# CFGpp-diffusion/CFGpp

Measured on NVIDIA B200. Metric: images/sec (device-timed) SDXL 1024x1024 NFE=50 ddim_cfg++, higher is better.
Workload: dtype f16

## Files before the change

cfgpp_b200/csrc/attention.cu:

```cuda
#include <cmath>
#include <cstdlib>
#include <cstring>

#include "attention.cuh"
#include "common.cuh"

namespace cfgpp {

void attn_configure();
void xattn_configure();
bool xattn_applicable(const AttnOp& op);
void run_xattn_op(const AttnOp& op, cudaStream_t stream);
void attn_persist_configure();
bool attn_persist_applicable(const AttnOp& op);
void run_attn_persist_op(const AttnOp& op, cudaStream_t stream);

namespace {

constexpr int BQ = 128;
constexpr int BKV = 128;
constexpr int ATOM_BYTES = 128 * 64 * 2;
constexpr int kThreads = 384;
constexpr uint32_t TMEM_COLS = 512;
constexpr float kRescaleThreshold = 8.0f;
constexpr int kDefaultPoly = 0;
constexpr int kDefaultRowsumMma = 0;
constexpr int kDefaultPbuf = 1;

template <int HD, int NQT, int KS, bool RS = false, int PB = 1>
struct ACfg {
  static constexpr int NA = HD / 64;
  static constexpr int TILE_BYTES = NA * ATOM_BYTES;
  static constexpr int P_BYTES = 2 * ATOM_BYTES;
  static constexpr int OW = HD + (RS ? 16 : 0);
  static constexpr int SMEM_BYTES =
      TILE_BYTES * (NQT + 2 * KS) + P_BYTES * NQT * PB + (RS ? ATOM_BYTES : 0) + 1024 + 256;
  static constexpr uint32_t O_COL = NQT * 128;
  static_assert(!RS || HD == 64, "the ones column is implemented for head dim 64");
  static_assert(NQT * 128 + NQT * OW <= 512, "TMEM overflow");
  static_assert(SMEM_BYTES <= 232448, "shared memory overflow");
};

template <int HD, int NQT, int KS, int POLY, bool RS, int PB>
__global__ void __launch_bounds__(kThreads, 1)
attn_kernel(const AttnParams p, const __grid_constant__ CUtensorMap map_q, const __grid_constant__ CUtensorMap map_k,
            const __grid_constant__ CUtensorMap map_v) {
  using A = ACfg<HD, NQT, KS, RS, PB>;
  constexpr int OW = A::OW;
  constexpr int TILE_BYTES = A::TILE_BYTES;
  constexpr int NA = A::NA;
  constexpr uint32_t O_COL = A::O_COL;
  extern __shared__ uint8_t smem_raw[];
  const uint32_t raw_addr = smem_u32(smem_raw);
  uint8_t* smem = smem_raw + (((raw_addr + 1023u) & ~1023u) - raw_addr);
  uint8_t* sQ = smem;
  uint8_t* sK = sQ + NQT * TILE_BYTES;
  uint8_t* sV = sK + KS * TILE_BYTES;
  uint8_t* sP = sV + KS * TILE_BYTES;
  uint8_t* sOnes = sP + NQT * PB * A::P_BYTES;
  uint64_t* bars = reinterpret_cast<uint64_t*>(sOnes + (RS ? ATOM_BYTES : 0));
  uint64_t* q_full = bars;
  uint64_t* k_full = q_full + 2;
  uint64_t* k_empty = k_full + KS;
  uint64_t* v_full = k_empty + KS;
  uint64_t* v_empty = v_full + KS;
  uint64_t* s_full = v_empty + KS;
  uint64_t* s_free = s_full + 2;
  uint64_t* p_full = s_free + 2;
  uint64_t* pv_done = p_full + 2 * PB;
  uint32_t* tmem_ptr_smem = reinterpret_cast<uint32_t*>(pv_done + 2 * PB);

  const int warp_idx = threadIdx.x >> 5;
  const int lane = threadIdx.x & 31;
  const int q0 = blockIdx.x * NQT * BQ;
  const int head = blockIdx.y;
  const int batch = blockIdx.z;
  const int n_tiles = (p.Nkv + BKV - 1) / BKV;
  const int n_qt = (NQT == 2 && q0 + BQ < p.Nq) ? 2 : 1;

  if (warp_idx == 0 && lane == 0) {
    tma_prefetch_desc(&map_q);
    tma_prefetch_desc(&map_k);
    tma_prefetch_desc(&map_v);
  }
  if (warp_idx == 1 && lane == 0) {
    for (int i = 0; i < 2; ++i) {
      mbar_init(&q_full[i], 1);
      mbar_init(&s_full[i], 1);
      mbar_init(&s_free[i], 128);
      for (int b = 0; b < PB; ++b) {
        mbar_init(&p_full[i * PB + b], 128);
        mbar_init(&pv_done[i * PB + b], 1);
      }
    }
    for (int i = 0; i < KS; ++i) {
      mbar_init(&k_full[i], 1);
      mbar_init(&k_empty[i], n_qt);
      mbar_init(&v_full[i], 1);
      mbar_init(&v_empty[i], n_qt);
    }
    fence_barrier_init();
  }
  if (warp_idx == 2) {
    tmem_alloc(tmem_ptr_smem, TMEM_COLS);
    tmem_relinquish();
  }
  if constexpr (RS) {
    if (warp_idx == 3) {
      for (int k = lane; k < 128; k += 32) {
        uint4* rowp = reinterpret_cast<uint4*>(sOnes + k * 128);
#pragma unroll
        for (int ch = 0; ch < 8; ++ch) rowp[ch] = make_uint4(ch == (k & 7) ? 0x00003C00u : 0u, 0u, 0u, 0u);
      }
      fence_proxy_async_smem();
    }
  }
  tc_fence_before();
  __syncthreads();
  tc_fence_after();
  const uint32_t tmem_base = *tmem_ptr_smem;
  pdl_launch_dependents();
  pdl_wait();

  if (warp_idx == 0) {
    if (lane == 0) {
      for (int qt = 0; qt < n_qt; ++qt) {
        mbar_arrive_expect_tx(&q_full[qt], TILE_BYTES);
        for (int a = 0; a < NA; ++a)
          tma_load_3d(sQ + qt * TILE_BYTES + a * ATOM_BYTES, &map_q, &q_full[qt], head * HD + a * 64, q0 + qt * BQ,
                      batch);
      }
      for (int j = 0; j < n_tiles; ++j) {
        const int s = j % KS;
        const uint32_t ph = (j / KS) & 1;
        mbar_wait(&k_empty[s], ph ^ 1);
        mbar_arrive_expect_tx(&k_full[s], TILE_BYTES);
        for (int a = 0; a < NA; ++a)
          tma_load_3d(sK + s * TILE_BYTES + a * ATOM_BYTES, &map_k, &k_full[s], head * HD + a * 64, j * BKV, batch);
        mbar_wait(&v_empty[s], ph ^ 1);
        mbar_arrive_expect_tx(&v_full[s], TILE_BYTES);
        for (int a = 0; a < NA; ++a)
          tma_load_3d(sV + s * TILE_BYTES + a * ATOM_BYTES, &map_v, &v_full[s], head * HD + a * 64, j * BKV, batch);
      }
    }
  } else if (warp_idx == 1) {
    if (lane == 0) {
      constexpr uint32_t idesc_qk = make_idesc_f16(128, BKV, 0, 0);
      constexpr uint32_t idesc_pv = make_idesc_f16(128, OW, 0, 1);
      auto issue_qk = [&](int qt, int j) {
#pragma unroll
        for (int a = 0; a < NA; ++a) {
          const uint64_t q_desc = make_sdesc_sw128(smem_u32(sQ + qt * TILE_BYTES + a * ATOM_BYTES), 1024, 0);
          const uint64_t k_desc = make_sdesc_sw128(smem_u32(sK + (j % KS) * TILE_BYTES + a * ATOM_BYTES), 1024, 0);
#pragma unroll
          for (int k = 0; k < 4; ++k)
            umma_f16(tmem_base + qt * BKV, q_desc + 2 * k, k_desc + 2 * k, idesc_qk, (a | k) != 0 ? 1u : 0u);
        }
        umma_commit(&s_full[qt]);
      };
      auto issue_pv = [&](int qt, int j) {
        const uint32_t v_addr = smem_u32(sV + (j % KS) * TILE_BYTES);
        const uint64_t v_desc = make_sdesc_sw128(v_addr, 1024, RS ? (smem_u32(sOnes) - v_addr) : ATOM_BYTES);
        const uint8_t* pbuf = sP + (qt * PB + (j % PB)) * A::P_BYTES;
#pragma unroll
        for (int k = 0; k < BKV / 16; ++k) {
          const uint64_t p_desc = make_sdesc_sw128(smem_u32(pbuf + (k >> 2) * ATOM_BYTES), 1024, 0) + 2 * (k & 3);
          umma_f16(tmem_base + O_COL + qt * OW, p_desc, v_desc + 128 * k, idesc_pv, (j | k) != 0 ? 1u : 0u);
        }
        umma_commit(&pv_done[qt * PB + (j % PB)]);
      };
      for (int qt = 0; qt < n_qt; ++qt) mbar_wait(&q_full[qt], 0);
      mbar_wait(&k_full[0], 0);
      tc_fence_after();
      for (int qt = 0; qt < n_qt; ++qt) {
        issue_qk(qt, 0);
// ... 16 lines not shown
            progressed = true;
          }
          j = next_qk[qt];
          if (j < n_tiles && mbar_try_wait(&s_free[qt], (j - 1) & 1) && mbar_try_wait(&k_full[j % KS], (j / KS) & 1)) {
            tc_fence_after();
            issue_qk(qt, j);
            umma_commit(&k_empty[j % KS]);
            ++next_qk[qt];
            --remaining;
            progressed = true;
          }
        }
        if (progressed) {
          t_start = clock64();
        } else if (clock64() - t_start > 4000000000LL) {
          printf("cfgpp: attention MMA issuer stalled (block %d,%d,%d)\n", blockIdx.x, blockIdx.y, blockIdx.z);
          __trap();
        }
      }
    }
  } else if (warp_idx >= 4) {
    const int qt = (warp_idx - 4) >> 2;
    if (qt < n_qt) {
      const int qw = warp_idx & 3;
      const int row = qw * 32 + lane;
      const uint32_t lane_off = static_cast<uint32_t>(qw * 32) << 16;
      const uint32_t s_addr = tmem_base + qt * BKV + lane_off;
      const uint32_t o_addr = tmem_base + O_COL + qt * OW + lane_off;
      uint8_t* prow0 = sP + qt * PB * A::P_BYTES + row * 128;
      const float c = p.scale_log2e;
      float m_ref = -INFINITY, l_run = 0.f;

      for (int j = 0; j < n_tiles; ++j) {
        const int valid = p.Nkv - j * BKV;
        mbar_wait(&s_full[qt], j & 1);
        tc_fence_after();
        uint32_t s[128];
#pragma unroll
        for (int g = 0; g < 4; ++g) tmem_ld_x32(s_addr + g * 32, *reinterpret_cast<uint32_t(*)[32]>(&s[g * 32]));
        tmem_ld_wait();
        tc_fence_before();
        mbar_arrive(&s_free[qt]);
        if (valid < BKV) {
#pragma unroll
          for (int i = 0; i < 128; ++i)
            if (i >= valid) s[i] = 0xff800000u;
        }
        float mxc[8];
#pragma unroll
        for (int k8 = 0; k8 < 8; ++k8) mxc[k8] = fmaxf(__uint_as_float(s[k8]), __uint_as_float(s[8 + k8]));
#pragma unroll
        for (int i = 16; i < 128; i += 16) {
#pragma unroll
          for (int k8 = 0; k8 < 8; ++k8) mxc[k8] = fmax3(mxc[k8], __uint_as_float(s[i + k8]), __uint_as_float(s[i + 8 + k8]));
        }
        const float mx = fmax3(fmax3(mxc[0], mxc[1], mxc[2]), fmax3(mxc[3], mxc[4], mxc[5]), fmaxf(mxc[6], mxc[7]));
        float alpha = 1.0f;
        bool need = false;
        if (j == 0) {
          m_ref = mx;
        } else if ((mx - m_ref) * c > kRescaleThreshold) {
          alpha = fast_exp2((m_ref - mx) * c);
          m_ref = mx;
          need = true;
        }
        uint8_t* prow = prow0 + (j % PB) * A::P_BYTES;
        if (j >= PB) {
          mbar_wait(&pv_done[qt * PB + (j % PB)], ((j - PB) / PB) & 1);
          tc_fence_after();
        }
        if (j > 0 && __any_sync(0xffffffffu, need)) {
          if constexpr (PB > 1) {
            mbar_wait(&pv_done[qt * PB + ((j - 1) % PB)], ((j - 1) / PB) & 1);
            tc_fence_after();
          }
#pragma unroll 1
          for (int h = 0; h < OW / 16; ++h) {
            uint32_t o[16];
            tmem_ld_x16(o_addr + h * 16, o);
            tmem_ld_wait();
#pragma unroll
            for (int d = 0; d < 16; ++d) o[d] = __float_as_uint(__uint_as_float(o[d]) * alpha);
            tmem_st_x16(o_addr + h * 16, o);
          }
          tmem_st_wait();
          l_run *= alpha;
        }
        const float mc = m_ref * c;
        float rs0 = 0.f, rs1 = 0.f;
#pragma unroll
        for (int g = 0; g < 16; ++g) {
          uint32_t pk[4];
#pragma unroll
          for (int e = 0; e < 4; ++e) {
            const float x0 = __uint_as_float(s[g * 8 + 2 * e]) * c - mc;
            const float x1 = __uint_as_float(s[g * 8 + 2 * e + 1]) * c - mc;
            constexpr int kP = POLY > 0 ? POLY : 1;
            const bool poly0 = POLY > 0 && ((g * 8 + 2 * e) % kP) == kP - 1;
            const bool poly1 = POLY > 0 && ((g * 8 + 2 * e + 1) % kP) == kP - 1;
            const float p0 = poly0 ? exp2_poly(x0) : fast_exp2(x0);
            const float p1 = poly1 ? exp2_poly(x1) : fast_exp2(x1);
            if constexpr (!RS) {
              rs0 += p0;
              rs1 += p1;
            }
            pk[e] = pack_half2(p0, p1);
          }
          const int half_idx = g >> 3;
          const int ch = (g & 7) ^ (row & 7);
          *reinterpret_cast<uint4*>(prow + half_idx * ATOM_BYTES + ch * 16) = make_uint4(pk[0], pk[1], pk[2], pk[3]);
        }
        l_run += rs0 + rs1;
        tc_fence_before();
        fence_proxy_async_smem();
        mbar_arrive(&p_full[qt * PB + (j % PB)]);
      }
      mbar_wait(&pv_done[qt * PB + ((n_tiles - 1) % PB)], ((n_tiles - 1) / PB) & 1);
      tc_fence_after();
      if constexpr (RS) {
        uint32_t lcol[16];
        tmem_ld_x16(o_addr + HD, lcol);
        tmem_ld_wait();
        l_run = __uint_as_float(lcol[0]);
      }
      const float inv_l = 1.0f / l_run;
      const int qrow = q0 + qt * BQ + row;
      __half* dst = p.out + (static_cast<size_t>(batch) * p.Nq + qrow) * p.ldo + head * HD;
#pragma unroll 1
      for (int h = 0; h < HD / 32; ++h) {
        uint32_t o[32];
        tmem_ld_x32(o_addr + h * 32, o);
        tmem_ld_wait();
        if (qrow < p.Nq) {
#pragma unroll
          for (int i = 0; i < 4; ++i) {
            uint4 w;
            w.x = pack_half2(__uint_as_float(o[8 * i + 0]) * inv_l, __uint_as_float(o[8 * i + 1]) * inv_l);
            w.y = pack_half2(__uint_as_float(o[8 * i + 2]) * inv_l, __uint_as_float(o[8 * i + 3]) * inv_l);
            w.z = pack_half2(__uint_as_float(o[8 * i + 4]) * inv_l, __uint_as_float(o[8 * i + 5]) * inv_l);
            w.w = pack_half2(__uint_as_float(o[8 * i + 6]) * inv_l, __uint_as_float(o[8 * i + 7]) * inv_l);
            reinterpret_cast<uint4*>(dst + h * 32)[i] = w;
          }
        }
      }
    }
  }

  tc_fence_before();
  __syncthreads();
  if (warp_idx == 2) {
    tc_fence_after();
    tmem_dealloc(tmem_base, TMEM_COLS);
  }
}

CUtensorMap make_head_map(const __half* base, int ld, int B, int N, int cols) {
  uint64_t dims[3] = {(uint64_t)cols, (uint64_t)N, (uint64_t)B};
  uint64_t strides[2] = {(uint64_t)ld * 2, (uint64_t)N * ld * 2};
  uint32_t box[3] = {64, 128, 1};
  return make_tmap_f16(base, 3, dims, strides, box);
}

template <int HD, int NQT, int KS, int POLY = 0, bool RS = false, int PB = 1>
void configure_one() {
  CFGPP_CHECK_CUDA(cudaFuncSetAttribute(attn_kernel<HD, NQT, KS, POLY, RS, PB>,
                                        cudaFuncAttributeMaxDynamicSharedMemorySize,
                                        ACfg<HD, NQT, KS, RS, PB>::SMEM_BYTES));
}

template <int HD, int NQT, int KS, int POLY = 0, bool RS = false, int PB = 1>
void launch(const AttnOp& op, cudaStream_t stream) {
  dim3 grid((op.p.Nq + NQT * BQ - 1) / (NQT * BQ), op.p.H, op.p.B);
  launch_pdl(attn_kernel<HD, NQT, KS, POLY, RS, PB>, grid, dim3(kThreads), ACfg<HD, NQT, KS, RS, PB>::SMEM_BYTES, stream,
             op.p, op.map_q, op.map_k, op.map_v);
}

int attn_pbuf() {
  static int v = -1;
  if (v < 0) {
    const char* e = std::getenv("CFGPP_ATTN_PBUF");
    v = e ? atoi(e) : kDefaultPbuf;
    if (v != 1 && v != 2) v = kDefaultPbuf;
  }
  return v;
}

bool attn_rowsum_mma() {
  static int v = -1;
  if (v < 0) {
    const char* e = std::getenv("CFGPP_ATTN_ROWSUM_MMA");
    v = e ? (e[0] == '1' ? 1 : 0) : kDefaultRowsumMma;
  }
  return v == 1;
}

int attn_poly() {
  static int v = -1;
  if (v < 0) {
    const char* e = std::getenv("CFGPP_ATTN_POLY");
    v = e ? atoi(e) : kDefaultPoly;
    if (v != 0 && v != 8 && v != 4 && v != 3) v = kDefaultPoly;
  }
  return v;
}

}

int attn_padded_head_dim(int head_dim) { return ((head_dim + 63) / 64) * 64; }

AttnOp make_attn_op(const __half* q, int ldq, const __half* k, int ldk, const __half* v, int ldv, __half* out,
                    int ldo, int B, int H, int Nq, int Nkv, int head_dim) {
  AttnOp op{};
  CFGPP_REQUIRE(Nkv >= 1 && Nq >= 1, "empty attention");
  CFGPP_REQUIRE(ldo % 8 == 0, "ldo must be a multiple of 8");
  CFGPP_REQUIRE(head_dim >= 8 && head_dim <= 192, "attention supports head_dim <= 192");
  const int hdp = attn_padded_head_dim(head_dim);
  op.hd_pad = hdp;
  op.head_dim = head_dim;
  op.p.B = B; op.p.H = H; op.p.Nq = Nq; op.p.Nkv = Nkv; op.p.ldo = ldo; op.p.out = out;
  op.p.scale_log2e = (1.0f / sqrtf(static_cast<float>(head_dim))) * 1.4426950408889634f;
  op.map_q = make_head_map(q, ldq, B, Nq, H * hdp);
  op.map_k = make_head_map(k, ldk, B, Nkv, H * hdp);
  op.map_v = make_head_map(v, ldv, B, Nkv, H * hdp);
  return op;
}

void attn_configure() {
  static bool done = false;
  if (done) return;
  configure_one<64, 2, 3>();
  configure_one<64, 2, 3, 8>();
  configure_one<64, 2, 3, 4>();
  configure_one<64, 2, 3, 3>();
  configure_one<64, 2, 3, 0, true>();
  configure_one<64, 2, 2, 0, false, 2>();
  configure_one<128, 1, 2>();
  configure_one<192, 1, 1>();
  xattn_configure();
  attn_persist_configure();
  done = true;
}

void run_attn_op(const AttnOp& op, cudaStream_t stream) {
  attn_configure();
  static const bool no_x = [] {
    const char* e = std::getenv("CFGPP_NO_XATTN");
    return e != nullptr && e[0] == '1';
  }();
  if (!no_x && xattn_applicable(op)) return run_xattn_op(op, stream);
  static const bool use_p = [] {
    const char* e = std::getenv("CFGPP_PATTN");
    return e != nullptr && e[0] == '1';
  }();
  if (use_p && attn_persist_applicable(op)) return run_attn_persist_op(op, stream);
  attn_configure();
  switch (op.hd_pad) {
    case 64:
      if (attn_pbuf() == 2) return launch<64, 2, 2, 0, false, 2>(op, stream);
      if (attn_rowsum_mma()) return launch<64, 2, 3, 0, true>(op, stream);
      switch (attn_poly()) {
        case 8: return launch<64, 2, 3, 8>(op, stream);
        case 4: return launch<64, 2, 3, 4>(op, stream);
        case 3: return launch<64, 2, 3, 3>(op, stream);
        default: return launch<64, 2, 3>(op, stream);
      }
    case 128: return launch<128, 1, 2>(op, stream);
    case 192: return launch<192, 1, 1>(op, stream);
    default: throw Error(-1, "unsupported padded head dim");
  }
}

}
```

cfgpp_b200/csrc/attention.cuh:

```cuda
#pragma once
#include "host.h"

namespace cfgpp {

struct AttnParams {
  int B, H, Nq, Nkv;
  int ldo;
  __half* out;
  float scale_log2e;
};

struct AttnOp {
  CUtensorMap map_q, map_k, map_v;
  AttnParams p;
  int hd_pad;
  int head_dim;
  double flops() const { return 4.0 * p.B * p.H * (double)p.Nq * p.Nkv * head_dim; }
};

int attn_padded_head_dim(int head_dim);
AttnOp make_attn_op(const __half* q, int ldq, const __half* k, int ldk, const __half* v, int ldv, __half* out,
                    int ldo, int B, int H, int Nq, int Nkv, int head_dim = 64);
void run_attn_op(const AttnOp& op, cudaStream_t stream);

}
```

cfgpp_b200/csrc/capi_ops.cu:

```cuda
#include "capi_util.h"
#include "attention.cuh"
#include "gemm.cuh"
#include "ops.cuh"
#include "../../include/cfgpp_b200.h"

using namespace cfgpp;

extern "C" {

CFGPP_API int cfgpp_op_linear(const void* a, int lda, const void* a2, int lda2, int k_split, const void* w, int M,
                              int N, int K, const void* bias, const void* addend, int ld_add,
                              int add_rows_per_group, void* out, int ldc, int geglu, int force_bn, void* stream) {
  return guarded([&] {
    GemmOp op = make_linear_op((const __half*)a, lda, (const __half*)a2, lda2, k_split, (const __half*)w, M, N, K,
                               (const __half*)bias, (const __half*)addend, ld_add, add_rows_per_group, (__half*)out,
                               ldc, geglu != 0, force_bn);
    run_gemm_op(op, (cudaStream_t)stream);
  });
}

CFGPP_API int cfgpp_dbg_linear_timeline(const void* a, int lda, const void* w, int M, int N, int K, const void* bias,
                                        const void* addend, void* out, int force_bn, int iters,
                                        unsigned long long* host_out , int* grid_out, void* stream) {
  return guarded([&] {
// ... 3 lines not shown
    CFGPP_CHECK_CUDA(cudaMalloc(&d, sizeof(unsigned long long) * 16 * op.grid));
    CFGPP_CHECK_CUDA(cudaMemset(d, 0, sizeof(unsigned long long) * 16 * op.grid));
    op.p.timeline = d;
    for (int i = 0; i < iters; ++i) run_gemm_op(op, (cudaStream_t)stream);
    CFGPP_CHECK_CUDA(cudaStreamSynchronize((cudaStream_t)stream));
    CFGPP_CHECK_CUDA(cudaMemcpy(host_out, d, sizeof(unsigned long long) * 16 * op.grid, cudaMemcpyDeviceToHost));
    *grid_out = op.grid;
    cudaFree(d);
  });
}

CFGPP_API int cfgpp_op_conv3x3(const void* x, int B, int H, int W, int Cin, const void* w, int Cout, const void* bias,
                               const void* addend, int ld_add, int add_rows_per_group, void* out, int force_bn,
                               void* stream) {
  return guarded([&] {
    GemmOp op = make_conv3x3_op((const __half*)x, B, H, W, Cin, (const __half*)w, Cout, (const __half*)bias,
                                (const __half*)addend, ld_add, add_rows_per_group, (__half*)out, force_bn);
    run_gemm_op(op, (cudaStream_t)stream);
  });
}

CFGPP_API int cfgpp_op_conv3x3_s2(const void* x, int B, int H, int W, int Cin, const void* w, int Cout, const void* bias,
                                  int pad, void* out, void* stream) {
  return guarded([&] {
    GemmOp op = make_conv3x3_op((const __half*)x, B, H, W, Cin, (const __half*)w, Cout, (const __half*)bias, nullptr, 0, 1,
                                (__half*)out, 0, 2, pad);
    run_gemm_op(op, (cudaStream_t)stream);
  });
}

CFGPP_API int cfgpp_op_attention(const void* q, int ldq, const void* k, int ldk, const void* v, int ldv, void* out,
                                 int ldo, int B, int H, int Nq, int Nkv, int head_dim, void* stream) {
  return guarded([&] {
    AttnOp op = make_attn_op((const __half*)q, ldq, (const __half*)k, ldk, (const __half*)v, ldv, (__half*)out, ldo,
                             B, H, Nq, Nkv, head_dim);
    run_attn_op(op, (cudaStream_t)stream);
  });
}

CFGPP_API int cfgpp_op_groupnorm(const void* x1, int C1, const void* x2, int C2, int B, int HW, const void* gamma,
                                 const void* beta, float eps, int silu, void* out, void* stream) {
  return guarded([&] {
    float* partial = nullptr;
    CFGPP_CHECK_CUDA(cudaMalloc(&partial, gn_partial_floats(B, HW) * sizeof(float)));
    try {
      run_groupnorm((const __half*)x1, C1, (const __half*)x2, C2, B, HW, (const __half*)gamma, (const __half*)beta,
                    eps, silu != 0, partial, (__half*)out, (cudaStream_t)stream);
    } catch (...) {
      cudaFree(partial);
      throw;
    }
    CFGPP_CHECK_CUDA(cudaStreamSynchronize((cudaStream_t)stream));
    cudaFree(partial);
  });
}

CFGPP_API int cfgpp_op_layernorm(const void* x, int M, int C, const void* gamma, const void* beta, float eps,
                                 void* out, void* stream) {
  return guarded([&] {
    run_layernorm((const __half*)x, M, C, (const __half*)gamma, (const __half*)beta, eps, (__half*)out,
                  (cudaStream_t)stream);
  });
}

CFGPP_API int cfgpp_op_cfgpp_step(const void* eps_uc, const void* eps_c, int n, int method, int state_dtype,
                                  const cfgpp_step_coef* coef_host, void* z, void* aux, void* z0t_out,
                                  const void* noise_dev, void* stream) {
  return guarded([&] {
// ... 24 lines not shown
```

cfgpp_b200/csrc/common.cuh:

```cuda
#pragma once
#include <cuda.h>
#include <cuda_fp16.h>
#include <cuda_runtime.h>
#include <stdint.h>
#include <stdio.h>

namespace cfgpp {

#define CFGPP_DEVICE __device__ __forceinline__

CFGPP_DEVICE uint32_t smem_u32(const void* p) {
  return static_cast<uint32_t>(__cvta_generic_to_shared(p));
}

CFGPP_DEVICE void pdl_launch_dependents() { asm volatile("griddepcontrol.launch_dependents;" ::: "memory"); }
CFGPP_DEVICE void pdl_wait() { asm volatile("griddepcontrol.wait;" ::: "memory"); }

CFGPP_DEVICE void mbar_init(uint64_t* bar, uint32_t count) {
  asm volatile("mbarrier.init.shared::cta.b64 [%0], %1;" ::"r"(smem_u32(bar)), "r"(count));
}
CFGPP_DEVICE void fence_barrier_init() {
  asm volatile("fence.mbarrier_init.release.cluster;" ::: "memory");
}
CFGPP_DEVICE void mbar_arrive_expect_tx(uint64_t* bar, uint32_t bytes) {
// ... 272 lines not shown
  float e;
  asm("ex2.approx.ftz.f32 %0, %1;" : "=f"(e) : "f"(-az * az * 1.4426950408889634f));
  float p = 1.061405429f;
  p = fmaf(p, t, -1.453152027f);
  p = fmaf(p, t, 1.421413741f);
  p = fmaf(p, t, -0.284496736f);
  p = fmaf(p, t, 0.254829592f);
  const float q = p * t * e;
  return 0.5f * x * (x >= 0.f ? 2.0f - q : q);
}

CFGPP_DEVICE float fast_exp2(float x) {
  float y;
  asm("ex2.approx.ftz.f32 %0, %1;" : "=f"(y) : "f"(x));
  return y;
}

CFGPP_DEVICE float exp2_poly(float x) {
  x = fmaxf(x, -126.0f);
  const float t = x + 12582912.0f;
  const float r = x - (t - 12582912.0f);
  float p = 0.0551716648042202f;
  p = fmaf(p, r, 0.2426111251115799f);
  p = fmaf(p, r, 0.6932609677314758f);
  p = fmaf(p, r, 0.9999280571937561f);
  return __int_as_float(__float_as_int(p) + (__float_as_int(t) << 23));
}
CFGPP_DEVICE float fmax3(float a, float b, float c) {
  float d;
  asm("max.f32 %0, %1, %2, %3;" : "=f"(d) : "f"(a), "f"(b), "f"(c));
  return d;
}

CFGPP_DEVICE uint32_t pack_half2(float a, float b) {
  __half2 h = __floats2half2_rn(a, b);
  return *reinterpret_cast<uint32_t*>(&h);
}

}
```

cfgpp_b200/csrc/unet.cu:

```cuda
#include "unet.cuh"

#include <algorithm>
#include <cstdlib>
#include <cstring>

#include "common.cuh"

namespace cfgpp {

namespace {

__global__ void f32_to_f16_kernel(const float* __restrict__ in, __half* __restrict__ out, size_t n) {
  for (size_t i = blockIdx.x * static_cast<size_t>(blockDim.x) + threadIdx.x; i < n;
       i += static_cast<size_t>(gridDim.x) * blockDim.x)
    out[i] = __float2half_rn(in[i]);
}

__global__ void pack_conv3x3_kernel(const __half* __restrict__ in, __half* __restrict__ out, int Cout, int Cin) {
  const size_t n = static_cast<size_t>(Cout) * Cin * 9;
  for (size_t i = blockIdx.x * static_cast<size_t>(blockDim.x) + threadIdx.x; i < n;
       i += static_cast<size_t>(gridDim.x) * blockDim.x) {
    const int ci = i % Cin;
    const size_t t = i / Cin;
    const int tap = t % 9;
// ... 363 lines not shown
  add_gemm(prefix + ".conv1", make_conv3x3_op(normp, bnb_, H, W, Cin, packed_conv3x3(prefix + ".conv1.weight"), Cout,
                                              plain(prefix + ".conv1.bias"), temb_all_ + static_cast<size_t>(brow0_) * temb_total_ + temb_off, temb_total_, HW,
                                              h1p));
  add_step(prefix + ".norm2+silu", [=](cudaStream_t st) {
    run_groupnorm(h1p, Cout, nullptr, 0, NB, HW, g2, b2, eps, true, partial, normp, st);
  }, 2);
  const __half* residual = x1p;
  if (Cin != Cout) {
    add_gemm(prefix + ".conv_shortcut",
             make_linear_op(x1p, C1, x2p, C2, C1, plain(prefix + ".conv_shortcut.weight"), static_cast<int>(M), Cout,
                            Cin, plain(prefix + ".conv_shortcut.bias"), nullptr, 0, 1, s_sc->p, Cout, false));
    residual = s_sc->p;
  }
  add_gemm(prefix + ".conv2", make_conv3x3_op(normp, bnb_, H, W, Cout, packed_conv3x3(prefix + ".conv2.weight"), Cout,
                                              plain(prefix + ".conv2.bias"), residual, Cout, 1, out));
  return Act{out, Cout};
}

Unet::Act Unet::build_transformer(const std::string& prefix, Act x, int H, int W, int layers, int heads) {
  const int C = x.C;
  const int HW = H * W;
  const int Mi = bnb_ * HW;
  const size_t M = static_cast<size_t>(Mi);
  const int D = d_.cross_attention_dim;
  CFGPP_REQUIRE(C % heads == 0 && C / heads <= 192,
                "attention supports head_dim <= 192 (got " + std::to_string(C / std::max(heads, 1)) + ") at " + prefix);
  const int hd = C / heads;
  const int hdp = attn_padded_head_dim(hd);
  const int Cp = heads * hdp;
  Scratch* s_norm = scratch(btag_ + "norm", M * C);
  Scratch* s_tok = scratch(btag_ + "tokens", M * C);
  Scratch* s_qkv = scratch(btag_ + "qkv", M * 3 * Cp);
  Scratch* s_attn = scratch(btag_ + "attn", M * Cp);
  Scratch* s_q = scratch(btag_ + "q", M * Cp);
  Scratch* s_ff = scratch(btag_ + "ff", M * 4 * C);
  Scratch* s_stats[3];
  for (int i = 0; i < 3; ++i)
    s_stats[i] = scratch(btag_ + "lnstats" + std::to_string(i), static_cast<size_t>(32) * M * 2 * 2);
  __half* out = g_dry ? nullptr : alloc_act(M * C);
  const int Mkv = bnb_ * n_ctx_;
  if (g_dry) {
    raw(prefix + ".norm.weight"); raw(prefix + ".norm.bias"); raw(prefix + ".proj_in.weight");
    raw(prefix + ".proj_in.bias"); raw(prefix + ".proj_out.weight"); raw(prefix + ".proj_out.bias");
    for (int k = 0; k < layers; ++k) {
      const std::string b = prefix + ".transformer_blocks." + std::to_string(k);
      for (const char* n : {".norm1.weight", ".norm1.bias", ".norm2.weight", ".norm2.bias", ".norm3.weight",
                            ".norm3.bias", ".attn1.to_q.weight", ".attn1.to_k.weight", ".attn1.to_v.weight",
                            ".attn1.to_out.0.weight", ".attn1.to_out.0.bias", ".attn2.to_q.weight",
                            ".attn2.to_k.weight", ".attn2.to_v.weight", ".attn2.to_out.0.weight",
                            ".attn2.to_out.0.bias", ".ff.net.0.proj.weight", ".ff.net.0.proj.bias",
                            ".ff.net.2.weight", ".ff.net.2.bias"})
        raw(b + n);
      workspace_bytes_ += static_cast<size_t>(Mkv) * 2 * Cp * sizeof(__half);
    }
    workspace_bytes_ += M * C * sizeof(__half);
    return Act{nullptr, C};
  }
  const int NB = bnb_;
  float* partial = bgn_partial_;
  __half *normp = s_norm->p, *tok = s_tok->p, *qkv = s_qkv->p, *attn = s_attn->p, *qb = s_q->p, *ff = s_ff->p;
  const bool fold = !lnfold_disabled();
  float* stats[3] = {nullptr, nullptr, nullptr};
  int parts[3] = {0, 0, 0};
  if (fold)
    for (int i = 0; i < 3; ++i) stats[i] = reinterpret_cast<float*>(s_stats[i]->p);
  auto producer = [&](const std::function<GemmOp(int)>& make, int slot) {
// ... 23 lines not shown
  };
  {
    const __half *g = plain(prefix + ".norm.weight"), *b = plain(prefix + ".norm.bias");
    const __half* xp = x.p;
    add_step(prefix + ".norm", [=](cudaStream_t st) {
      run_groupnorm(xp, C, nullptr, 0, NB, HW, g, b, 1e-6f, false, partial, normp, st);
    }, 2);
  }
  add_gemm(prefix + ".proj_in", producer([&](int bn) {
             return make_linear_op(normp, C, nullptr, 0, 0, plain(prefix + ".proj_in.weight"), Mi, C, C,
                                   plain(prefix + ".proj_in.bias"), nullptr, 0, 1, tok, C, false, bn);
           }, 0));
  for (int k = 0; k < layers; ++k) {
    const std::string b = prefix + ".transformer_blocks." + std::to_string(k);
    auto add_ln = [&](const std::string& n) {
      const __half *g = plain(b + n + ".weight"), *be = plain(b + n + ".bias");
      add_step(b + n, [=](cudaStream_t st) { run_layernorm(tok, Mi, C, g, be, 1e-5f, normp, st); });
    };
    __half* wqkv = packed_heads_rows({b + ".attn1.to_q.weight", b + ".attn1.to_k.weight", b + ".attn1.to_v.weight"},
                                     heads, hd, hdp);
    if (fold) {
      const FoldedLN f = folded_ln(b + ".attn1.qkv", wqkv, 3 * Cp, C, b + ".norm1", nullptr);
      add_gemm(b + ".attn1.to_qkv(+norm1)",
               consumer(make_linear_op(tok, C, nullptr, 0, 0, f.w, Mi, 3 * Cp, C, nullptr, nullptr, 0, 1, qkv, 3 * Cp, false),
                        f, 0),
               2.0 * Mi * 3.0 * C * C);
    } else {
      add_ln(".norm1");
      add_gemm(b + ".attn1.to_qkv",
               make_linear_op(normp, C, nullptr, 0, 0, wqkv, Mi, 3 * Cp, C, nullptr, nullptr, 0, 1, qkv, 3 * Cp, false),
               2.0 * Mi * 3.0 * C * C);
    }
    add_attn(b + ".attn1.sdpa",
             make_attn_op(qkv, 3 * Cp, qkv + Cp, 3 * Cp, qkv + 2 * Cp, 3 * Cp, attn, Cp, bnb_, heads, HW, HW, hd));
    add_gemm(b + ".attn1.to_out", producer([&](int bn) {
               return make_linear_op(attn, Cp, nullptr, 0, 0,
                                     packed_heads_cols(b + ".attn1.to_out.0.weight", heads, hd, hdp), Mi, C, Cp,
                                     plain(b + ".attn1.to_out.0.bias"), tok, C, 1, tok, C, false, bn);
             }, 1),
             2.0 * Mi * static_cast<double>(C) * C);
    __half* wq2 = packed_heads_rows({b + ".attn2.to_q.weight"}, heads, hd, hdp);
    if (fold) {
      const FoldedLN f = folded_ln(b + ".attn2.q", wq2, Cp, C, b + ".norm2", nullptr);
      add_gemm(b + ".attn2.to_q(+norm2)",
               consumer(make_linear_op(tok, C, nullptr, 0, 0, f.w, Mi, Cp, C, nullptr, nullptr, 0, 1, qb, Cp, false), f, 1),
               2.0 * Mi * static_cast<double>(C) * C);
    } else {
      add_ln(".norm2");
      add_gemm(b + ".attn2.to_q",
               make_linear_op(normp, C, nullptr, 0, 0, wq2, Mi, Cp, C, nullptr, nullptr, 0, 1, qb, Cp, false),
               2.0 * Mi * static_cast<double>(C) * C);
    }
    __half* kv = alloc_act(static_cast<size_t>(Mkv) * 2 * Cp);
    {
      __half* wkv = packed_heads_rows({b + ".attn2.to_k.weight", b + ".attn2.to_v.weight"}, heads, hd, hdp);
      std::vector<PlanStep>* save = cur_plan_;
      cur_plan_ = &prompt_plan_;
      add_gemm(b + ".attn2.to_kv",
               make_linear_op(ctx_copy_ + static_cast<size_t>(brow0_) * n_ctx_ * D, D, nullptr, 0, 0, wkv, Mkv, 2 * Cp, D,
                              nullptr, nullptr, 0, 1, kv, 2 * Cp, false),
               2.0 * Mkv * 2.0 * C * D);
      cur_plan_ = save;
    }
    add_attn(b + ".attn2.sdpa", make_attn_op(qb, Cp, kv, 2 * Cp, kv + Cp, 2 * Cp, attn, Cp, bnb_, heads, HW, n_ctx_, hd));
    add_gemm(b + ".attn2.to_out", producer([&](int bn) {
               return make_linear_op(attn, Cp, nullptr, 0, 0,
                                     packed_heads_cols(b + ".attn2.to_out.0.weight", heads, hd, hdp), Mi, C, Cp,
                                     plain(b + ".attn2.to_out.0.bias"), tok, C, 1, tok, C, false, bn);
             }, 2),
             2.0 * Mi * static_cast<double>(C) * C);
    __half* wg = packed_geglu(b + ".ff.net.0.proj.weight", false);
    __half* bg = packed_geglu(b + ".ff.net.0.proj.bias", true);
    if (fold) {
      const FoldedLN f = folded_ln(b + ".ff.geglu", wg, 8 * C, C, b + ".norm3", bg);
      add_gemm(b + ".ff.geglu(+norm3)",
               consumer(make_linear_op(tok, C, nullptr, 0, 0, f.w, Mi, 8 * C, C, nullptr, nullptr, 0, 1, ff, 4 * C, true), f, 2));
    } else {
      add_ln(".norm3");
      add_gemm(b + ".ff.geglu",
               make_linear_op(normp, C, nullptr, 0, 0, wg, Mi, 8 * C, C, bg, nullptr, 0, 1, ff, 4 * C, true));
    }
    add_gemm(b + ".ff.out", producer([&](int bn) {
               return make_linear_op(ff, 4 * C, nullptr, 0, 0, plain(b + ".ff.net.2.weight"), Mi, C, 4 * C,
                                     plain(b + ".ff.net.2.bias"), tok, C, 1, tok, C, false, bn);
             }, 0));
  }
  add_gemm(prefix + ".proj_out", make_linear_op(tok, C, nullptr, 0, 0, plain(prefix + ".proj_out.weight"), Mi, C, C,
                                                plain(prefix + ".proj_out.bias"), x.p, C, 1, out, C, false));
  return Act{out, C};
}

Unet::Act Unet::build_downsample(const std::string& prefix, Act x, int H, int W) {
  const int C = x.C;
  const int Ho = H / 2, Wo = W / 2;
  const size_t Mo = static_cast<size_t>(bnb_) * Ho * Wo;
  static const bool use_im2col = [] {
    const char* e = getenv("CFGPP_NO_S2TMA");
// ... 69 lines not shown
  graph_valid_ = false;
  B_ = batch; NB_ = 2 * batch; H_ = h_lat; W_ = w_lat;
  const int L = d_.num_levels;
  const int C0 = d_.block_out_channels[0];
  const int TE = time_embed_dim_;

  temb_order_.clear();
  temb_total_ = 0;
  std::vector<std::string> temb_w_keys, temb_b_keys;
  auto reg_resnet = [&](const std::string& prefix, int Cout) {
    temb_order_.push_back({prefix, temb_total_});
    temb_total_ += Cout;
    temb_w_keys.push_back(prefix + ".time_emb_proj.weight");
    temb_b_keys.push_back(prefix + ".time_emb_proj.bias");
  };
  for (int i = 0; i < L; ++i)
    for (int j = 0; j < d_.layers_per_block; ++j)
      reg_resnet("down_blocks." + std::to_string(i) + ".resnets." + std::to_string(j), d_.block_out_channels[i]);
  reg_resnet("mid_block.resnets.0", d_.block_out_channels[L - 1]);
  reg_resnet("mid_block.resnets.1", d_.block_out_channels[L - 1]);
  for (int i = 0; i < L; ++i)
    for (int j = 0; j < d_.layers_per_block + 1; ++j)
      reg_resnet("up_blocks." + std::to_string(i) + ".resnets." + std::to_string(j), d_.block_out_channels[L - 1 - i]);
  auto temb_off = [&](const std::string& prefix) {
    for (auto& p : temb_order_)
      if (p.first == prefix) return p.second;
    throw Error(-11, "internal: unknown resnet " + prefix);
  };

  for (int pass = 0; pass < 2; ++pass) {
    g_dry = (pass == 0);
    if (!g_dry) {
      workspace_bytes_ = 0;
      for (auto& kv : scratch_) kv.second->p = alloc_act(kv.second->need);
      gn_partial_ = static_cast<float*>(alloc_bytes(static_cast<size_t>(NB_) * 128 * 64 * sizeof(float)));
      t_sin_ = alloc_act(C0);
      t_h1_ = alloc_act(TE);
      emb_ = alloc_act(static_cast<size_t>(NB_) * TE);
      semb_ = alloc_act(static_cast<size_t>(NB_) * TE);
      temb_all_ = alloc_act(static_cast<size_t>(NB_) * temb_total_);
      ctx_copy_ = alloc_act(static_cast<size_t>(NB_) * n_ctx_ * d_.cross_attention_dim);
      if (has_aug_) {
        add_in_ = alloc_act(static_cast<size_t>(NB_) * d_.projection_class_embeddings_input_dim);
        add_h1_ = alloc_act(static_cast<size_t>(NB_) * TE);
        aug_emb_ = alloc_act(static_cast<size_t>(NB_) * TE);
        pooled_copy_ = alloc_act(static_cast<size_t>(NB_) * d_.pooled_dim);
        time_ids_copy_ = static_cast<float*>(alloc_bytes(static_cast<size_t>(NB_) * 6 * sizeof(float)));
      }
      cur_state_ = static_cast<StepState*>(alloc_bytes(sizeof(StepState)));
      step_counter_ = static_cast<int*>(alloc_bytes(sizeof(int)));
      step_table_ = static_cast<StepState*>(alloc_bytes(sizeof(StepState) * 1024));
      const size_t lat = static_cast<size_t>(B_) * 4 * H_ * W_;
      z_state_ = alloc_bytes(lat * sizeof(float));
      aux_state_ = alloc_bytes(lat * sizeof(float));
      z0t_state_ = alloc_bytes(lat * sizeof(float));
      noise_slot_ = static_cast<const __half**>(alloc_bytes(sizeof(__half*)));
      CFGPP_CHECK_CUDA(cudaMemcpy(noise_slot_, &noise_buf_, sizeof(__half*), cudaMemcpyHostToDevice));
      fwd_eps_uc_ = alloc_act(lat);
      fwd_eps_c_ = alloc_act(lat);
      temb_w_all_ = packed_cat_rows(temb_w_keys);
      temb_b_all_ = packed_cat_rows(temb_b_keys);
      conv_in_w_ = plain("conv_in.weight");
      conv_in_b_ = plain("conv_in.bias");
      conv_out_w_ = packed_conv3x3("conv_out.weight");
      conv_out_b_ = plain("conv_out.bias");
    } else {
      for (const char* k : {"conv_in.weight", "conv_in.bias", "conv_out.weight", "conv_out.bias",
// ... 360 lines not shown
```

Before: 1.176.

## Split KV range for tail-wave attention tiles and use packed f32x2 math

Flattens the attention grid to 1D and, when the last wave only partly fills the SMs, splits the KV range of the leftover tiles across several CTAs. Each piece writes partial O, max and sum to a float workspace, and the last-arriving CTA, found via an atomic counter, merges them into the half-precision output. The softmax scaling, the rowsum and the O rescale also switch to packed fma/add/mul f32x2 instructions. This adds workspace traffic, counter synchronisation and a merge pass for the split tiles in exchange for better SM occupancy in the final wave.

```diff
diff --git a/cfgpp_b200/csrc/attention.cu b/cfgpp_b200/csrc/attention.cu
--- a/cfgpp_b200/csrc/attention.cu
+++ b/cfgpp_b200/csrc/attention.cu
@@ -26,6 +26,11 @@
 constexpr int kDefaultPoly = 0;
 constexpr int kDefaultRowsumMma = 0;
 constexpr int kDefaultPbuf = 1;
+constexpr int kMaxSplit = 8;
+#ifndef CFGPP_ATTN_MIN_PIECE
+#define CFGPP_ATTN_MIN_PIECE 2
+#endif
+constexpr int kMinPieceTiles = CFGPP_ATTN_MIN_PIECE;
 
 template <int HD, int NQT, int KS, bool RS = false, int PB = 1>
 struct ACfg {
@@ -41,7 +46,7 @@
   static_assert(SMEM_BYTES <= 232448, "shared memory overflow");
 };
 
-template <int HD, int NQT, int KS, int POLY, bool RS, int PB>
+template <int HD, int NQT, int KS, int POLY, bool RS, int PB, bool PK>
 __global__ void __launch_bounds__(kThreads, 1)
 attn_kernel(const AttnParams p, const __grid_constant__ CUtensorMap map_q, const __grid_constant__ CUtensorMap map_k,
             const __grid_constant__ CUtensorMap map_v) {
@@ -72,10 +77,21 @@
 
   const int warp_idx = threadIdx.x >> 5;
   const int lane = threadIdx.x & 31;
-  const int q0 = blockIdx.x * NQT * BQ;
-  const int head = blockIdx.y;
-  const int batch = blockIdx.z;
-  const int n_tiles = (p.Nkv + BKV - 1) / BKV;
+  const int n_pairs = (p.Nq + NQT * BQ - 1) / (NQT * BQ);
+  const int n_kv = (p.Nkv + BKV - 1) / BKV;
+  int item = blockIdx.x, piece = -1, kv_begin = 0, kv_end = n_kv;
+  if (item >= p.n_full) {
+    const int r = item - p.n_full;
+    item = p.n_full + r / p.split;
+    piece = r % p.split;
+    kv_begin = piece * n_kv / p.split;
+    kv_end = (piece + 1) * n_kv / p.split;
+  }
+  const int q0 = (item % n_pairs) * NQT * BQ;
+  const int head = (item / n_pairs) % p.H;
+  const int batch = item / (n_pairs * p.H);
+  const int kv0 = kv_begin * BKV;
+  const int n_tiles = kv_end - kv_begin;
   const int n_qt = (NQT == 2 && q0 + BQ < p.Nq) ? 2 : 1;
 
   if (warp_idx == 0 && lane == 0) {
@@ -136,11 +152,13 @@
         mbar_wait(&k_empty[s], ph ^ 1);
         mbar_arrive_expect_tx(&k_full[s], TILE_BYTES);
         for (int a = 0; a < NA; ++a)
-          tma_load_3d(sK + s * TILE_BYTES + a * ATOM_BYTES, &map_k, &k_full[s], head * HD + a * 64, j * BKV, batch);
+          tma_load_3d(sK + s * TILE_BYTES + a * ATOM_BYTES, &map_k, &k_full[s], head * HD + a * 64, kv0 + j * BKV,
+                      batch);
         mbar_wait(&v_empty[s], ph ^ 1);
         mbar_arrive_expect_tx(&v_full[s], TILE_BYTES);
         for (int a = 0; a < NA; ++a)
-          tma_load_3d(sV + s * TILE_BYTES + a * ATOM_BYTES, &map_v, &v_full[s], head * HD + a * 64, j * BKV, batch);
+          tma_load_3d(sV + s * TILE_BYTES + a * ATOM_BYTES, &map_v, &v_full[s], head * HD + a * 64, kv0 + j * BKV,
+                      batch);
       }
     }
   } else if (warp_idx == 1) {
@@ -223,7 +241,7 @@
       float m_ref = -INFINITY, l_run = 0.f;
 
       for (int j = 0; j < n_tiles; ++j) {
-        const int valid = p.Nkv - j * BKV;
+        const int valid = p.Nkv - kv0 - j * BKV;
         mbar_wait(&s_full[qt], j & 1);
         tc_fence_after();
         uint32_t s[128];
@@ -271,29 +289,51 @@
             tmem_ld_x16(o_addr + h * 16, o);
             tmem_ld_wait();
 #pragma unroll
-            for (int d = 0; d < 16; ++d) o[d] = __float_as_uint(__uint_as_float(o[d]) * alpha);
+            for (int d = 0; d < 16; d += 2) {
+              float2 od = make_float2(__uint_as_float(o[d]), __uint_as_float(o[d + 1]));
+              if constexpr (PK) {
+                od = fmul2(od, make_float2(alpha, alpha));
+              } else {
+                od.x *= alpha;
+                od.y *= alpha;
+              }
+              o[d] = __float_as_uint(od.x);
+              o[d + 1] = __float_as_uint(od.y);
+            }
             tmem_st_x16(o_addr + h * 16, o);
           }
           tmem_st_wait();
           l_run *= alpha;
         }
         const float mc = m_ref * c;
-        float rs0 = 0.f, rs1 = 0.f;
+        float2 rs = make_float2(0.f, 0.f);
 #pragma unroll
         for (int g = 0; g < 16; ++g) {
           uint32_t pk[4];
 #pragma unroll
           for (int e = 0; e < 4; ++e) {
-            const float x0 = __uint_as_float(s[g * 8 + 2 * e]) * c - mc;
-            const float x1 = __uint_as_float(s[g * 8 + 2 * e + 1]) * c - mc;
+            const float2 sp = make_float2(__uint_as_float(s[g * 8 + 2 * e]), __uint_as_float(s[g * 8 + 2 * e + 1]));
+            float x0, x1;
+            if constexpr (PK) {
+              const float2 x = ffma2(sp, make_float2(c, c), make_float2(-mc, -mc));
+              x0 = x.x;
+              x1 = x.y;
+            } else {
+              x0 = sp.x * c - mc;
+              x1 = sp.y * c - mc;
+            }
             constexpr int kP = POLY > 0 ? POLY : 1;
             const bool poly0 = POLY > 0 && ((g * 8 + 2 * e) % kP) == kP - 1;
             const bool poly1 = POLY > 0 && ((g * 8 + 2 * e + 1) % kP) == kP - 1;
             const float p0 = poly0 ? exp2_poly(x0) : fast_exp2(x0);
             const float p1 = poly1 ? exp2_poly(x1) : fast_exp2(x1);
             if constexpr (!RS) {
-              rs0 += p0;
-              rs1 += p1;
+              if constexpr (PK) {
+                rs = fadd2(rs, make_float2(p0, p1));
+              } else {
+                rs.x += p0;
+                rs.y += p1;
+              }
             }
             pk[e] = pack_half2(p0, p1);
           }
@@ -301,7 +341,7 @@
           const int ch = (g & 7) ^ (row & 7);
           *reinterpret_cast<uint4*>(prow + half_idx * ATOM_BYTES + ch * 16) = make_uint4(pk[0], pk[1], pk[2], pk[3]);
         }
-        l_run += rs0 + rs1;
+        l_run += rs.x + rs.y;
         tc_fence_before();
         fence_proxy_async_smem();
         mbar_arrive(&p_full[qt * PB + (j % PB)]);
@@ -314,23 +354,45 @@
         tmem_ld_wait();
         l_run = __uint_as_float(lcol[0]);
       }
-      const float inv_l = 1.0f / l_run;
-      const int qrow = q0 + qt * BQ + row;
-      __half* dst = p.out + (static_cast<size_t>(batch) * p.Nq + qrow) * p.ldo + head * HD;
+      if (piece >= 0) {
+        float* slot = p.ws + static_cast<size_t>((blockIdx.x - p.n_full) * 2 + qt) * (HD + 2) * BQ;
 #pragma unroll 1
-      for (int h = 0; h < HD / 32; ++h) {
-        uint32_t o[32];
-        tmem_ld_x32(o_addr + h * 32, o);
-        tmem_ld_wait();
-        if (qrow < p.Nq) {
-#pragma unroll
-          for (int i = 0; i < 4; ++i) {
-            uint4 w;
-            w.x = pack_half2(__uint_as_float(o[8 * i + 0]) * inv_l, __uint_as_float(o[8 * i + 1]) * inv_l);
-            w.y = pack_half2(__uint_as_float(o[8 * i + 2]) * inv_l, __uint_as_float(o[8 * i + 3]) * inv_l);
-            w.z = pack_half2(__uint_as_float(o[8 * i + 4]) * inv_l, __uint_as_float(o[8 * i + 5]) * inv_l);
-            w.w = pack_half2(__uint_as_float(o[8 * i + 6]) * inv_l, __uint_as_float(o[8 * i + 7]) * inv_l);
-            reinterpret_cast<uint4*>(dst + h * 32)[i] = w;
+        for (int h = 0; h < HD / 32; ++h) {
+          uint32_t o[32];
+          tmem_ld_x32(o_addr + h * 32, o);
+          tmem_ld_wait();
+#pragma unroll
+          for (int i = 0; i < 32; ++i) slot[(h * 32 + i) * BQ + row] = __uint_as_float(o[i]);
+        }
+        slot[HD * BQ + row] = m_ref;
+        slot[(HD + 1) * BQ + row] = l_run;
+        __threadfence();
+      } else {
+        const float inv_l = 1.0f / l_run;
+        const int qrow = q0 + qt * BQ + row;
+        __half* dst = p.out + (static_cast<size_t>(batch) * p.Nq + qrow) * p.ldo + head * HD;
+#pragma unroll 1
+        for (int h = 0; h < HD / 32; ++h) {
+          uint32_t o[32];
+          tmem_ld_x32(o_addr + h * 32, o);
+          tmem_ld_wait();
+          if (qrow < p.Nq) {
+            uint32_t w[16];
+#pragma unroll
+            for (int i = 0; i < 16; ++i) {
+              float2 od = make_float2(__uint_as_float(o[2 * i]), __uint_as_float(o[2 * i + 1]));
+              if constexpr (PK) {
+                od = fmul2(od, make_float2(inv_l, inv_l));
+              } else {
+                od.x *= inv_l;
+                od.y *= inv_l;
+              }
+              w[i] = pack_half2(od.x, od.y);
+            }
+#pragma unroll
+            for (int i = 0; i < 4; ++i)
+              reinterpret_cast<uint4*>(dst + h * 32)[i] =
+                  make_uint4(w[4 * i], w[4 * i + 1], w[4 * i + 2], w[4 * i + 3]);
           }
         }
       }
@@ -343,6 +405,66 @@
     tc_fence_after();
     tmem_dealloc(tmem_base, TMEM_COLS);
   }
+  if (piece >= 0) {
+    volatile uint32_t* last_flag = tmem_ptr_smem + 1;
+    if (threadIdx.x == 128) {
+      int* cnt = p.cnt + (item - p.n_full);
+      const bool last = atomicAdd(cnt, 1) == p.split - 1;
+      if (last) *cnt = 0;
+      *last_flag = last ? 1u : 0u;
+    }
+    __syncthreads();
+    if (*last_flag != 0u && warp_idx >= 4) {
+      __threadfence();
+      const int qt = (warp_idx - 4) >> 2;
+      const int row = (warp_idx & 3) * 32 + lane;
+      const int qrow = q0 + qt * BQ + row;
+      if (qt < n_qt && qrow < p.Nq) {
+        const float c = p.scale_log2e;
+        const size_t slot_floats = static_cast<size_t>(HD + 2) * BQ;
+        const float* base = p.ws + static_cast<size_t>((item - p.n_full) * p.split * 2 + qt) * slot_floats;
+        float mk[kMaxSplit], w[kMaxSplit];
+        float m = -INFINITY;
+#pragma unroll
+        for (int k = 0; k < kMaxSplit; ++k) {
+          if (k < p.split) {
+            mk[k] = __ldcg(base + 2 * k * slot_floats + HD * BQ + row);
+            m = fmaxf(m, mk[k]);
+          }
+        }
+        float l = 0.f;
+#pragma unroll
+        for (int k = 0; k < kMaxSplit; ++k) {
+          if (k < p.split) {
+            w[k] = fast_exp2((mk[k] - m) * c);
+            l += __ldcg(base + 2 * k * slot_floats + (HD + 1) * BQ + row) * w[k];
+          }
+        }
+        const float inv_l = 1.0f / l;
+        __half* dst = p.out + (static_cast<size_t>(batch) * p.Nq + qrow) * p.ldo + head * HD;
+#pragma unroll 1
+        for (int h = 0; h < HD / 32; ++h) {
+          float acc[32];
+#pragma unroll
+          for (int i = 0; i < 32; ++i) acc[i] = 0.f;
+#pragma unroll
+          for (int k = 0; k < kMaxSplit; ++k) {
+            if (k < p.split) {
+              const float* src = base + 2 * k * slot_floats + (h * 32) * BQ + row;
+#pragma unroll
+              for (int i = 0; i < 32; ++i) acc[i] = fmaf(__ldcg(src + i * BQ), w[k], acc[i]);
+            }
+          }
+          uint32_t pk[16];
+#pragma unroll
+          for (int i = 0; i < 16; ++i) pk[i] = pack_half2(acc[2 * i] * inv_l, acc[2 * i + 1] * inv_l);
+#pragma unroll
+          for (int i = 0; i < 4; ++i)
+            reinterpret_cast<uint4*>(dst + h * 32)[i] = make_uint4(pk[4 * i], pk[4 * i + 1], pk[4 * i + 2], pk[4 * i + 3]);
+        }
+      }
+    }
+  }
 }
 
 CUtensorMap make_head_map(const __half* base, int ld, int B, int N, int cols) {
@@ -352,17 +474,18 @@
   return make_tmap_f16(base, 3, dims, strides, box);
 }
 
-template <int HD, int NQT, int KS, int POLY = 0, bool RS = false, int PB = 1>
+template <int HD, int NQT, int KS, int POLY = 0, bool RS = false, int PB = 1, bool PK = true>
 void configure_one() {
-  CFGPP_CHECK_CUDA(cudaFuncSetAttribute(attn_kernel<HD, NQT, KS, POLY, RS, PB>,
+  CFGPP_CHECK_CUDA(cudaFuncSetAttribute(attn_kernel<HD, NQT, KS, POLY, RS, PB, PK>,
                                         cudaFuncAttributeMaxDynamicSharedMemorySize,
                                         ACfg<HD, NQT, KS, RS, PB>::SMEM_BYTES));
 }
 
-template <int HD, int NQT, int KS, int POLY = 0, bool RS = false, int PB = 1>
+template <int HD, int NQT, int KS, int POLY = 0, bool RS = false, int PB = 1, bool PK = true>
 void launch(const AttnOp& op, cudaStream_t stream) {
-  dim3 grid((op.p.Nq + NQT * BQ - 1) / (NQT * BQ), op.p.H, op.p.B);
-  launch_pdl(attn_kernel<HD, NQT, KS, POLY, RS, PB>, grid, dim3(kThreads), ACfg<HD, NQT, KS, RS, PB>::SMEM_BYTES, stream,
+  const int items = (op.p.Nq + NQT * BQ - 1) / (NQT * BQ) * op.p.H * op.p.B;
+  dim3 grid(op.p.n_full + (items - op.p.n_full) * op.p.split);
+  launch_pdl(attn_kernel<HD, NQT, KS, POLY, RS, PB, PK>, grid, dim3(kThreads), ACfg<HD, NQT, KS, RS, PB>::SMEM_BYTES, stream,
              op.p, op.map_q, op.map_k, op.map_v);
 }
 
@@ -395,12 +518,58 @@
   return v;
 }
 
+struct TailSplit {
+  int n_full, split;
+};
+int attn_items(int B, int H, int Nq, int hdp) {
+  const int rows = (hdp == 64 ? 2 : 1) * BQ;
+  return (Nq + rows - 1) / rows * H * B;
+}
+TailSplit attn_tail_split(int B, int H, int Nq, int Nkv, int hdp) {
+  static const bool off = [] {
+    const char* e = std::getenv("CFGPP_ATTN_NO_TAILSPLIT");
+    return e != nullptr && e[0] == '1';
+  }();
+  const int items = attn_items(B, H, Nq, hdp);
+  if (off || hdp != 64) return {items, 1};
+  int dev = 0, sms = 0;
+  CFGPP_CHECK_CUDA(cudaGetDevice(&dev));
+  CFGPP_CHECK_CUDA(cudaDeviceGetAttribute(&sms, cudaDevAttrMultiProcessorCount, dev));
+  const int left = items % sms;
+  const int split = std::min(std::min(kMaxSplit, (Nkv + BKV - 1) / BKV / kMinPieceTiles), left > 0 ? sms / left : 0);
+  if (left == 0 || 3 * left >= 2 * sms || split < 2) return {items, 1};
+  return {items - left, split};
+}
+
+size_t attn_counters_bytes() {
+  int dev = 0, sms = 0;
+  CFGPP_CHECK_CUDA(cudaGetDevice(&dev));
+  CFGPP_CHECK_CUDA(cudaDeviceGetAttribute(&sms, cudaDevAttrMultiProcessorCount, dev));
+  return (sms * sizeof(int) + 255) / 256 * 256;
+}
+
+bool attn_scalar() {
+  static const bool v = [] {
+    const char* e = std::getenv("CFGPP_ATTN_SCALAR");
+    return e != nullptr && e[0] == '1';
+  }();
+  return v;
+}
+
 }
 
 int attn_padded_head_dim(int head_dim) { return ((head_dim + 63) / 64) * 64; }
 
+size_t attn_workspace_bytes(int B, int H, int Nq, int Nkv, int head_dim) {
+  const int hdp = attn_padded_head_dim(head_dim);
+  const TailSplit ts = attn_tail_split(B, H, Nq, Nkv, hdp);
+  if (ts.split == 1) return 0;
+  const size_t left = static_cast<size_t>(attn_items(B, H, Nq, hdp) - ts.n_full);
+  return attn_counters_bytes() + left * ts.split * 2 * (hdp + 2) * BQ * sizeof(float);
+}
+
 AttnOp make_attn_op(const __half* q, int ldq, const __half* k, int ldk, const __half* v, int ldv, __half* out,
-                    int ldo, int B, int H, int Nq, int Nkv, int head_dim) {
+                    int ldo, int B, int H, int Nq, int Nkv, int head_dim, void* workspace) {
   AttnOp op{};
   CFGPP_REQUIRE(Nkv >= 1 && Nq >= 1, "empty attention");
   CFGPP_REQUIRE(ldo % 8 == 0, "ldo must be a multiple of 8");
@@ -410,6 +579,14 @@
   op.head_dim = head_dim;
   op.p.B = B; op.p.H = H; op.p.Nq = Nq; op.p.Nkv = Nkv; op.p.ldo = ldo; op.p.out = out;
   op.p.scale_log2e = (1.0f / sqrtf(static_cast<float>(head_dim))) * 1.4426950408889634f;
+  const TailSplit ts = attn_tail_split(B, H, Nq, Nkv, hdp);
+  op.p.n_full = ts.n_full;
+  op.p.split = ts.split;
+  if (ts.split > 1) {
+    CFGPP_REQUIRE(workspace != nullptr, "attention: this shape needs attn_workspace_bytes() of workspace");
+    op.p.cnt = static_cast<int*>(workspace);
+    op.p.ws = reinterpret_cast<float*>(static_cast<char*>(workspace) + attn_counters_bytes());
+  }
   op.map_q = make_head_map(q, ldq, B, Nq, H * hdp);
   op.map_k = make_head_map(k, ldk, B, Nkv, H * hdp);
   op.map_v = make_head_map(v, ldv, B, Nkv, H * hdp);
@@ -420,6 +597,7 @@
   static bool done = false;
   if (done) return;
   configure_one<64, 2, 3>();
+  configure_one<64, 2, 3, 0, false, 1, false>();
   configure_one<64, 2, 3, 8>();
   configure_one<64, 2, 3, 4>();
   configure_one<64, 2, 3, 3>();
@@ -453,7 +631,9 @@
         case 8: return launch<64, 2, 3, 8>(op, stream);
         case 4: return launch<64, 2, 3, 4>(op, stream);
         case 3: return launch<64, 2, 3, 3>(op, stream);
-        default: return launch<64, 2, 3>(op, stream);
+        default:
+          if (attn_scalar()) return launch<64, 2, 3, 0, false, 1, false>(op, stream);
+          return launch<64, 2, 3>(op, stream);
       }
     case 128: return launch<128, 1, 2>(op, stream);
     case 192: return launch<192, 1, 1>(op, stream);
diff --git a/cfgpp_b200/csrc/attention.cuh b/cfgpp_b200/csrc/attention.cuh
--- a/cfgpp_b200/csrc/attention.cuh
+++ b/cfgpp_b200/csrc/attention.cuh
@@ -8,6 +8,9 @@
   int ldo;
   __half* out;
   float scale_log2e;
+  int n_full, split;
+  float* ws;
+  int* cnt;
 };
 
 struct AttnOp {
@@ -19,8 +22,9 @@
 };
 
 int attn_padded_head_dim(int head_dim);
+size_t attn_workspace_bytes(int B, int H, int Nq, int Nkv, int head_dim = 64);
 AttnOp make_attn_op(const __half* q, int ldq, const __half* k, int ldk, const __half* v, int ldv, __half* out,
-                    int ldo, int B, int H, int Nq, int Nkv, int head_dim = 64);
+                    int ldo, int B, int H, int Nq, int Nkv, int head_dim = 64, void* workspace = nullptr);
 void run_attn_op(const AttnOp& op, cudaStream_t stream);
 
 }
diff --git a/cfgpp_b200/csrc/capi_ops.cu b/cfgpp_b200/csrc/capi_ops.cu
--- a/cfgpp_b200/csrc/capi_ops.cu
+++ b/cfgpp_b200/csrc/capi_ops.cu
@@ -59,8 +59,20 @@
 CFGPP_API int cfgpp_op_attention(const void* q, int ldq, const void* k, int ldk, const void* v, int ldv, void* out,
                                  int ldo, int B, int H, int Nq, int Nkv, int head_dim, void* stream) {
   return guarded([&] {
+    static void* ws = nullptr;
+    static size_t ws_bytes = 0;
+    const size_t need = attn_workspace_bytes(B, H, Nq, Nkv, head_dim);
+    if (need > ws_bytes) {
+      CFGPP_CHECK_CUDA(cudaDeviceSynchronize());
+      if (ws) CFGPP_CHECK_CUDA(cudaFree(ws));
+      ws = nullptr;
+      ws_bytes = 0;
+      CFGPP_CHECK_CUDA(cudaMalloc(&ws, need));
+      CFGPP_CHECK_CUDA(cudaMemset(ws, 0, need));
+      ws_bytes = need;
+    }
     AttnOp op = make_attn_op((const __half*)q, ldq, (const __half*)k, ldk, (const __half*)v, ldv, (__half*)out, ldo,
-                             B, H, Nq, Nkv, head_dim);
+                             B, H, Nq, Nkv, head_dim, ws);
     run_attn_op(op, (cudaStream_t)stream);
   });
 }
diff --git a/cfgpp_b200/csrc/common.cuh b/cfgpp_b200/csrc/common.cuh
--- a/cfgpp_b200/csrc/common.cuh
+++ b/cfgpp_b200/csrc/common.cuh
@@ -328,6 +328,28 @@
   return d;
 }
 
+CFGPP_DEVICE float2 ffma2(float2 a, float2 b, float2 c) {
+  float2 d;
+  asm("{\n.reg .b64 a, b, c, d;\nmov.b64 a, {%2, %3};\nmov.b64 b, {%4, %5};\nmov.b64 c, {%6, %7};\n"
+      "fma.rn.f32x2 d, a, b, c;\nmov.b64 {%0, %1}, d;\n}"
+      : "=f"(d.x), "=f"(d.y) : "f"(a.x), "f"(a.y), "f"(b.x), "f"(b.y), "f"(c.x), "f"(c.y));
+  return d;
+}
+CFGPP_DEVICE float2 fadd2(float2 a, float2 b) {
+  float2 d;
+  asm("{\n.reg .b64 a, b, d;\nmov.b64 a, {%2, %3};\nmov.b64 b, {%4, %5};\n"
+      "add.rn.f32x2 d, a, b;\nmov.b64 {%0, %1}, d;\n}"
+      : "=f"(d.x), "=f"(d.y) : "f"(a.x), "f"(a.y), "f"(b.x), "f"(b.y));
+  return d;
+}
+CFGPP_DEVICE float2 fmul2(float2 a, float2 b) {
+  float2 d;
+  asm("{\n.reg .b64 a, b, d;\nmov.b64 a, {%2, %3};\nmov.b64 b, {%4, %5};\n"
+      "mul.rn.f32x2 d, a, b;\nmov.b64 {%0, %1}, d;\n}"
+      : "=f"(d.x), "=f"(d.y) : "f"(a.x), "f"(a.y), "f"(b.x), "f"(b.y));
+  return d;
+}
+
 CFGPP_DEVICE uint32_t pack_half2(float a, float b) {
   __half2 h = __floats2half2_rn(a, b);
   return *reinterpret_cast<uint32_t*>(&h);
diff --git a/cfgpp_b200/csrc/unet.cu b/cfgpp_b200/csrc/unet.cu
--- a/cfgpp_b200/csrc/unet.cu
+++ b/cfgpp_b200/csrc/unet.cu
@@ -419,6 +419,8 @@
   Scratch* s_tok = scratch(btag_ + "tokens", M * C);
   Scratch* s_qkv = scratch(btag_ + "qkv", M * 3 * Cp);
   Scratch* s_attn = scratch(btag_ + "attn", M * Cp);
+  Scratch* s_attn_ws = scratch(btag_ + "attn_ws", (std::max(attn_workspace_bytes(bnb_, heads, HW, HW, hd),
+                                                             attn_workspace_bytes(bnb_, heads, HW, n_ctx_, hd)) + 1) / 2);
   Scratch* s_q = scratch(btag_ + "q", M * Cp);
   Scratch* s_ff = scratch(btag_ + "ff", M * 4 * C);
   Scratch* s_stats[3];
@@ -508,7 +510,8 @@
                2.0 * Mi * 3.0 * C * C);
     }
     add_attn(b + ".attn1.sdpa",
-             make_attn_op(qkv, 3 * Cp, qkv + Cp, 3 * Cp, qkv + 2 * Cp, 3 * Cp, attn, Cp, bnb_, heads, HW, HW, hd));
+             make_attn_op(qkv, 3 * Cp, qkv + Cp, 3 * Cp, qkv + 2 * Cp, 3 * Cp, attn, Cp, bnb_, heads, HW, HW, hd,
+                          s_attn_ws->p));
     add_gemm(b + ".attn1.to_out", producer([&](int bn) {
                return make_linear_op(attn, Cp, nullptr, 0, 0,
                                      packed_heads_cols(b + ".attn1.to_out.0.weight", heads, hd, hdp), Mi, C, Cp,
@@ -538,7 +541,8 @@
                2.0 * Mkv * 2.0 * C * D);
       cur_plan_ = save;
     }
-    add_attn(b + ".attn2.sdpa", make_attn_op(qb, Cp, kv, 2 * Cp, kv + Cp, 2 * Cp, attn, Cp, bnb_, heads, HW, n_ctx_, hd));
+    add_attn(b + ".attn2.sdpa", make_attn_op(qb, Cp, kv, 2 * Cp, kv + Cp, 2 * Cp, attn, Cp, bnb_, heads, HW, n_ctx_, hd,
+                                             s_attn_ws->p));
     add_gemm(b + ".attn2.to_out", producer([&](int bn) {
                return make_linear_op(attn, Cp, nullptr, 0, 0,
                                      packed_heads_cols(b + ".attn2.to_out.0.weight", heads, hd, hdp), Mi, C, Cp,
@@ -674,7 +678,10 @@
     g_dry = (pass == 0);
     if (!g_dry) {
       workspace_bytes_ = 0;
-      for (auto& kv : scratch_) kv.second->p = alloc_act(kv.second->need);
+      for (auto& kv : scratch_) {
+        kv.second->p = alloc_act(kv.second->need);
+        CFGPP_CHECK_CUDA(cudaMemset(kv.second->p, 0, std::max<size_t>(kv.second->need, 8) * sizeof(__half)));
+      }
       gn_partial_ = static_cast<float*>(alloc_bytes(static_cast<size_t>(NB_) * 128 * 64 * sizeof(float)));
       t_sin_ = alloc_act(C0);
       t_h1_ = alloc_act(TE);
```

Measured after the change: 1.186 (median of 6 runs). About the same (+0.9%).
